# h2o/picotls

Hardware: AMD Instinct MI355X
Metric: AES-GCM seal+open GiB/s (device-resident), 16KiB & 1200B record batches (higher is better)
Workload: dtype u8

## Files before the change

### picotls_amd/csrc/engine/gcm_kernels.h

```cpp
#ifndef PTLS_MI355X_ENGINE_GCM_KERNELS_H
#define PTLS_MI355X_ENGINE_GCM_KERNELS_H

__device__ __forceinline__ u32 unit_mul(u32 steps, u32 log2, u32 cap)
{
    const u32 nc = (steps + (1u << log2) - 1) >> log2;
    return nc > cap ? (nc + cap - 1) / cap : 1u;
}
__device__ __forceinline__ u32 run_unit_cap(const BatchArgs &args)
{
    return args.w8_split ? (u32)W8_RUN_UNITS : (u32)CRUN_UNITS;
}

template <int FRAME = 0>
__device__ __forceinline__ bool record_ok(const BatchArgs &args, const ptls_mi355x_record_t &r)
{
    return r.len <= PTLS_MI355X_MAX_RECORD_LEN && gcm_aad_len<false, FRAME>(r) <= PTLS_MI355X_MAX_AAD_LEN &&
           r.key_idx < args.nkeys;
}

#ifndef SPREAD_MIN_BYTES
#define SPREAD_MIN_BYTES (512u << 10)
#endif
__device__ __forceinline__ bool spread_long(const BatchArgs &a, const ptls_mi355x_record_t &r)
{
// ... 517 lines not shown
            const u32 incl = carry + wave_incl_sum(np);
            if (t < 256) {
                plan[t] = incl - np;
                plan[256 + t] = e;
            }
            carry = (u32)__builtin_amdgcn_readlane((int)incl, 63);
        }
        if (lane == 0)
            plan[SPREAD_PLAN_CTL] = carry;
    }
    __syncthreads();
    const u32 P = __builtin_amdgcn_readfirstlane(plan[SPREAD_PLAN_CTL]);
    if (w >= P)
        return;
    auto piece_record = [&](u32 p) -> u32 {
        u32 lo = 0, hi = n;
        while (hi - lo > 1) {
            const u32 mid = (lo + hi) >> 1;
            if (plan[mid] <= p)
                lo = mid;
            else
                hi = mid;
        }
        return __builtin_amdgcn_readfirstlane(lo);
    };
    const u32 src8 = SPREAD_UNIT_STEPS == CHUNK_STEPS ? 8u : key_pow2_idx(3 + SPREAD_UNIT_LOG2);
    u32 loaded_key = args.multi_key ? args.recs[piece_record(w)].key_idx : 0u;
    if (wave >= EARLY_GHASH_WAVE)
        build_ghash_tables(lds, args.keys + loaded_key, 9, src8, 0, EARLY_GHASH_WAVE * 64, ENGINE_WG - EARLY_GHASH_WAVE * 64,
                           GHASH_WMASK);
    else
        build_aes_tables(lds, 0, EARLY_GHASH_WAVE * 64);
    __syncthreads();
    const u32 tsel_horner = 0x10000u + (u32)(G - 1) * GHASH_TABLE_BYTES, tsel_chunk = 0x10000u + 8u * GHASH_TABLE_BYTES;
    for (u32 p = w; p < P; p += nspare) {
        const u32 t = piece_record(p), s = p - plan[t], e = plan[256 + t], pbase = plan[t];
        const u32 np_t = (t + 1 < n ? plan[t + 1] : P) - pbase;
        const ptls_mi355x_record_t r = args.recs[t];
        const u32 kidx = args.multi_key ? __builtin_amdgcn_readfirstlane(r.key_idx) : 0u;
        if (kidx != loaded_key) {
            build_ghash_tables(lds, args.keys + kidx, 9, src8, 0, 0, 0, GHASH_WMASK);
            __syncthreads();
            loaded_key = kidx;
        }
        const KeyEntry *key = args.keys + kidx;
        u32 rk[NR + 1][4];
#pragma unroll
        for (int rr = 0; rr <= NR; ++rr)
#pragma unroll
            for (int c = 0; c < 4; ++c)
                rk[rr][c] = __builtin_amdgcn_readfirstlane(key->rk[rr][c]);
        const u32 iv0 = __builtin_amdgcn_readfirstlane(key->iv[0]), iv1 = __builtin_amdgcn_readfirstlane(key->iv[1]),
                  iv2 = __builtin_amdgcn_readfirstlane(key->iv[2]);
        const u32 steps = gcm_steps<OPEN, 0>(r), U = (steps + SPREAD_UNIT_STEPS - 1) / SPREAD_UNIT_STEPS;
        const u32 k0 = s << e, nu = min(U - k0, 1u << e);
        for (u32 uu0 = wave * 8; uu0 < nu; uu0 += ENGINE_WG / G) {
            const u32 lane = lane_here(), j = lane % G, uu = uu0 + lane / G, laneoff = (lane & 31) * 4;
            const bool valid = uu < nu;
            const u32 k = k0 + uu;
            u32 m_hi = 0, m_lo = 0;
            if (valid) {
                m_hi = steps - k * SPREAD_UNIT_STEPS;
                m_lo = k + 1 == U ? 0u : m_hi - SPREAD_UNIT_STEPS;
            }
            u32x4 acc;
            u32 okw;
            gcm_segment<NR, OPEN, 0, CT>(args, lds, rk, iv0, iv1, iv2, r, valid, m_lo, m_hi, j, laneoff, tsel_horner, acc, false,
                                         okw, false, CLDS_PART + 16u * uu);
            if (valid && j == G - 1)
                s_part[uu] = acc;
        }
        __syncthreads();
        const u32 mL = SPREAD_UNIT_LOG2 + e;
        const bool split = e >= 4 && mL <= 10 && (16u << e) <= GHASH_TABLE_BYTES;
        lds_u32x4 *s_sum = (lds_u32x4 *)(lds + CLDS_RUN1);
        const u32 tsel_ml = CLDS_PART + GHASH_TABLE_BYTES;
        if (split) {
            if (wave == 1)
                build_elem_table(lds, tsel_ml, u32x4{key->h[key_pow2_idx(mL)][0], key->h[key_pow2_idx(mL)][1],
                                                     key->h[key_pow2_idx(mL)][2], key->h[key_pow2_idx(mL)][3]}, 64, true);
            if (wave == 0) {
                const u32 lane = lane_here(), c = lane / G, L = 1u << (e - 3), ulo = c * L, uhi = min(ulo + L, nu);
                u32x4 g = {0, 0, 0, 0};
                if (ulo < uhi) {
                    g = s_part[uhi - 1];
                    for (u32 i = uhi - 1; i-- > ulo;)
                        g = gmul_combine(lds, g, tsel_chunk, lane) ^ s_part[i];
                }
                if (lane % G == 0)
                    s_sum[c] = g;
            }
            __syncthreads();
        }
        if (wave == 0) {
            const u32 lane = lane_here();
            u32x4 g;
            if (split) {
                g = s_sum[7];
                for (u32 c = 7; c-- > 0;)
                    g = gmul_combine(lds, g, tsel_ml, lane) ^ s_sum[c];
            } else {
                g = s_part[nu - 1];
                for (u32 i = nu - 1; i-- > 0;)
                    g = gmul_combine(lds, g, tsel_chunk, lane) ^ s_part[i];
            }
            if (lane == 0) {
                args.spread_part[pbase + s] = g;
                __threadfence();
                *s_flag = atomicAdd(args.spread_cnt + t, 1u) == np_t - 1;
            }
        }
        __syncthreads();
        if (*s_flag) {
            __threadfence();
            lds_u32x4 *s_m = (lds_u32x4 *)(lds + CLDS_PART + GHASH_TABLE_BYTES);
            const u32 m = 3 + SPREAD_UNIT_LOG2 + e, hi = m <= 10 ? key_pow2_idx(m) : 15u;
            if (threadIdx.x == 0)
                *s_m = u32x4{key->h[hi][0], key->h[hi][1], key->h[hi][2], key->h[hi][3]};
            __syncthreads();
            for (u32 i = 10; i < m; ++i) {
                build_elem_table(lds, CLDS_PART, *s_m);
                __syncthreads();
                const u32x4 sq = gmul_tab(lds, *s_m, CLDS_PART);
                __syncthreads();
                if (threadIdx.x == 0)
                    *s_m = sq;
                __syncthreads();
            }
            build_elem_table(lds, CLDS_PART, *s_m);
            __syncthreads();
            if (wave == 0) {
                const u32 lane = lane_here();
                const volatile u32x4 *vp = args.spread_part + pbase;
                u32x4 g = vp[np_t - 1];
                for (u32 i = np_t - 1; i-- > 0;)
                    g = gmul_tab(lds, g, CLDS_PART) ^ u32x4(vp[i]);
                if (lane == 0) {
                    if (OPEN) {
                        const u32x4 rt = *(const u32x4_u *)(args.in + r.in_off + r.len);
                        const u32x4 d = rt ^ g;
                        args.ok[t] = (d[0] | d[1] | d[2] | d[3]) == 0;
                    } else {
                        *(u32x4_u *)(args.out + r.out_off + r.len) = g;
                    }
                    args.spread_cnt[t] = 0;
                }
            }
        }
        __syncthreads();
    }
}


__device__ __noinline__ void w8_build_tables(lds_u8 *lds, const lds_u8 *keyp, u32 usrc, bool tree, u32 hpow)
{
    typedef __attribute__((address_space(3))) const KeyEntry lds_key_t;
    lds_key_t *key = (lds_key_t *)keyp;
    auto el = [&](u32 i) { return u32x4{key->h[i][0], key->h[i][1], key->h[i][2], key->h[i][3]}; };
    build_elem_table(lds, CLDS_PART, el(hpow), 0, false);
    build_elem_table(lds, W8_TAB_H, el(0), 64, !tree);
    if (tree)
        build_elem_table(lds, W8_TAB_COMB, el(1), 128, false);
    else if (usrc != 0xffffffffu)
        build_elem_table(lds, W8_TAB_COMB, el(usrc), 128, true);
    __syncthreads();
    build_h8_byte_table(lds, CLDS_PART);
    __syncthreads();
}

__device__ unsigned long long *g_kclock_buf;
__device__ unsigned int g_kclock_cap;
__device__ unsigned int g_kclock_n;

template <int NR, bool OPEN, int FRAME, bool CT = false, int EXT = 0>
__global__ __launch_bounds__(ENGINE_WG) __attribute__((amdgpu_waves_per_eu(ENGINE_WAVES_PER_SIMD, ENGINE_WAVES_PER_SIMD))) void gcm_chunked_kernel(BatchArgs args)
{
    extern __shared__ __attribute__((aligned(16))) uint8_t smem[];
    lds_u8 *lds = (lds_u8 *)smem;
    check_lds_base(smem);
    PROF_STAMP(tk);
    lds_u32x4 *s_part = (lds_u32x4 *)(lds + CLDS_PART);
    constexpr int G = ENGINE_G;
    constexpr int RPW = 64 / G;

    const u32 wave = threadIdx.x >> 6;
    const u32 tsel_horner = 0x10000u + (u32)(G - 1) * GHASH_TABLE_BYTES;
    constexpr bool W8K = EXT == 3 || EXT == 4 || EXT == 5;
    constexpr bool W8TREE = EXT == 3;
    const u32 tsel_chunk = W8K ? (u32)W8_TAB_COMB : 0x10000u + 8u * GHASH_TABLE_BYTES;

    const u64 n = args.nrecs, C = args.bounds != nullptr ? 0 : args.chunk;
    const u32 *slist = nullptr;
    u32 scnt = 0;
    if constexpr (W8TREE) {
        if (args.w8_split == 2 && args.w8_flags != nullptr) {
            scnt = args.w8_flags[(u64)blockIdx.x * W8_FLAG_WORDS];
            if (scnt == 0)
                return;
            if (scnt <= W8_SKIP_LIST)
                slist = args.w8_flags + (u64)blockIdx.x * W8_FLAG_WORDS + 1;
        }
    }
    unsigned long long *const kclock = ENGINE_HOOKS && blockIdx.x == 0 ? g_kclock_buf : nullptr;
    const u64 kc_t0 = kclock != nullptr ? __builtin_amdgcn_s_memtime() : 0ull;
    const u64 kc_r0 = kclock != nullptr ? __builtin_amdgcn_s_memrealtime() : 0ull;
    u32 skipped_w8 = 0;
    u32 runs_here = 0, g4_here = 0, mk_here = 0;
    constexpr bool SPREAD = FRAME == 0 && EXT == 1;
    if constexpr (SPREAD) {
        if (blockIdx.x >= n) {
            spread_pieces<NR, OPEN, CT>(args, blockIdx.x - (u32)n, gridDim.x - (u32)n);
            return;
        }
    }
    u64 beg = SPREAD ? (u64)blockIdx.x : args.bounds != nullptr ? args.bounds[blockIdx.x] : C != 0 ? min(n, (u64)blockIdx.x * C) : n * blockIdx.x / gridDim.x;
    u64 end = SPREAD ? (u64)blockIdx.x + 1 : args.bounds != nullptr ? args.bounds[blockIdx.x + 1] : C != 0 ? min(n, beg + C) : n * (blockIdx.x + 1) / gridDim.x;
    u64 cstart = beg;
    u32 sidx = 0;
    if constexpr (W8TREE) {
        if (slist != nullptr)
            beg = slist[0], end = slist[1];
    }
    u32 loaded_key = 0xffffffffu, loaded_usrc = 0xffffffffu;
    u32 loaded_w8 = 0;
    const ptls_mi355x_record_t *recs = args.recs;
    const u32 *perm = nullptr;
    if (args.perm_on != nullptr && *args.perm_on)
        recs = args.grouped, perm = args.perm;
    if (args.one_inline) {
        recs = (const ptls_mi355x_record_t *)(smem + CLDS_ONE);
        if (threadIdx.x < sizeof(ptls_mi355x_record_t) / 4)
            ((lds_u32 *)(lds + CLDS_ONE))[threadIdx.x] = ((const u32 *)&args.one)[threadIdx.x];
        __builtin_amdgcn_fence(__ATOMIC_SEQ_CST, "workgroup");
        __builtin_amdgcn_wave_barrier();
    }
    auto ok_at = [&](u64 i) -> u64 { return perm != nullptr ? (u64)perm[i] : i; };
    constexpr bool HPK = !OPEN && FRAME == 0 && EXT == 2;
    const bool with_hp = HPK && args.hp != nullptr;
    u64 hp_pos = 0;
    u32 hp_n = 0;
#define HP_PASS(p_, e_, tid_, nthr_)                                                                                    \
    do {                                                                                                                \
        if constexpr (HPK) {                                                                                            \
            if (args.hp_nr == 10)                                                                                       \
                hp_masks_pass<10>(args.hp, args.hp_keys, args.hp_nkeys, args.out, args.masks, (p_), (e_), perm, (tid_),  \
                                  (nthr_));                                                                             \
            else                                                                                                        \
                hp_masks_pass<14>(args.hp, args.hp_keys, args.hp_nkeys, args.out, args.masks, (p_), (e_), perm, (tid_),  \
                                  (nthr_));                                                                             \
        }                                                                                                               \
    } while (0)

    const bool early = !args.multi_key && !W8K;
    const u32 fixed_usrc = args.unit_log2 == CHUNK_LOG2 ? 8u : args.unit_log2 == 0 ? 7u : 8u + args.unit_log2;
    const bool early_combine = early && args.unit_log2 < CHUNK_LOG2;
    if (early && wave >= EARLY_GHASH_WAVE) {
        build_ghash_tables(lds, args.keys, early_combine ? 9u : 8u, fixed_usrc, 0, EARLY_GHASH_WAVE * 64,
                           ENGINE_WG - EARLY_GHASH_WAVE * 64, GHASH_WMASK);
    } else if (wave == 0) {
        if (beg < end)
            scan_run<OPEN, FRAME, true, EXT>(args, recs, beg, end, (lds_u32 *)(lds + CLDS_RUN0));
#if ENGINE_PROFILE
        if (threadIdx.x == 0)
            PROF_ADD(9, stamp() - tk), PROF_ADD(10, 1);
#endif
    } else {
        build_aes_tables(lds, 64, early ? EARLY_GHASH_WAVE * 64 : 0, W8K ? W8_AES_BASE : 0u);
#if ENGINE_PROFILE
        if (threadIdx.x == 64)
            PROF_ADD(8, stamp() - tk);
#endif
    }
    __syncthreads();

    if (early)
        loaded_key = 0, loaded_usrc = early_combine ? fixed_usrc : 0xffffffffu;

    u32 rb = 0;
    for (u64 pos = beg; pos < end;) {
        PROF_STAMP(t0);
        lds_u32 *rs = (lds_u32 *)(lds + (rb ? CLDS_RUN1 : CLDS_RUN0));
        lds_u32 *rs_next = (lds_u32 *)(lds + (rb ? CLDS_RUN0 : CLDS_RUN1));
        lds_u32 *s_ubase = rs + RUN_UBASE_OFF, *s_done = rs + RUN_DONE_OFF, *s_front = rs + RUN_FRONT_OFF;
        const u32 key_idx = __builtin_amdgcn_readfirstlane(rs[RC_KEY]);
        const u32 run_n = __builtin_amdgcn_readfirstlane(rs[RC_N]);
        const bool whole_run = __builtin_amdgcn_readfirstlane(rs[RC_WHOLE]);
        const u32 total_units = __builtin_amdgcn_readfirstlane(rs[RC_UNITS]);
        const u32 nhuge = __builtin_amdgcn_readfirstlane(rs[RC_HUGE]);
        const u32 mk_n = EXT == 5 ? __builtin_amdgcn_readfirstlane(rs[RC_MK]) : 0u;
        const u32 ulog2 = __builtin_amdgcn_readfirstlane(rs[RC_LOG2]), ustep = 1u << ulog2;
        const u32 usrc = ustep == CHUNK_STEPS ? 8u : ulog2 == 0 ? 7u : 8u + ulog2;
        const u32 nfull = total_units - run_n;
        const u64 run_end = pos + run_n;
        u64 nxt = run_end, nxt_end = end, nxt_cstart = cstart;
        if (C != 0 && run_end >= end) {
            nxt_cstart = cstart + (u64)gridDim.x * C;
            nxt = min(n, nxt_cstart);
            nxt_end = min(n, nxt_cstart + C);
        }
        if constexpr (W8TREE) {
            if (slist != nullptr) {
                if (sidx + 1 < scnt) {
                    nxt = slist[2 * sidx + 2];
                    nxt_end = slist[2 * sidx + 3];
                } else {
                    nxt = nxt_end = 0;
                }
                ++sidx;
            }
        }
        PROF_STAMP(t1);

        if (W8K && args.w8_split == 2) {
            const bool tree = whole_run &&
                              __builtin_amdgcn_readfirstlane(gcm_steps<OPEN, FRAME>(recs[pos]) >= W8_MIN_STEPS ? 1u : 0u) != 0;
            if (tree != W8TREE) {
                if constexpr (!W8TREE) {
                    const bool fits = end <= 0xffffffffull;
                    if (args.w8_flags != nullptr && threadIdx.x == 0 && skipped_w8 < W8_SKIP_LIST && fits) {
                        u32 *f = args.w8_flags + (u64)blockIdx.x * W8_FLAG_WORDS + 1 + 2 * skipped_w8;
                        f[0] = (u32)pos, f[1] = (u32)end;
                    }
                    skipped_w8 = fits ? skipped_w8 + 1 : W8_SKIP_LIST + 1;
                }
                if (wave == 0 && nxt < nxt_end)
                    scan_run<OPEN, FRAME, false, EXT>(args, recs, nxt, nxt_end, rs_next);
                __syncthreads();
                pos = nxt, end = nxt_end, cstart = nxt_cstart;
                rb ^= 1;
                continue;
            }
        }
        const bool whole = W8TREE || whole_run;
        if (key_idx >= args.nkeys) {
            if (OPEN)
                for (u64 t = pos + threadIdx.x; t < run_end; t += blockDim.x)
                    args.ok[ok_at(t)] = 0;
            if (wave == 0 && nxt < nxt_end)
                scan_run<OPEN, FRAME, false, EXT>(args, recs, nxt, nxt_end, rs_next);
            __syncthreads();
            if (with_hp) {
                if (hp_n != 0)
                    HP_PASS(hp_pos, hp_pos + hp_n, threadIdx.x, blockDim.x);
                HP_PASS(pos, run_end, threadIdx.x, blockDim.x);
                hp_n = 0;
            }
            pos = nxt, end = nxt_end, cstart = nxt_cstart;
            rb ^= 1;
            continue;
        }
        ++runs_here;
        typedef __attribute__((address_space(3))) const KeyEntry lds_key_t;
        lds_key_t *key = (lds_key_t *)(rs + RUN_KEY_OFF);
        constexpr bool w8run = W8K;
        const bool g4run = W8K && !W8TREE && whole;
        const u32 w8mode = !w8run ? 0u : W8TREE ? 2u : g4run ? 3u : 1u;
        const bool key_new = key_idx != loaded_key;
        if (mk_n != 0) {
            static_assert(ENGINE_WG >= 2 * MK_SLOTS * 128, "a table per 128 threads");
            const u32 t = threadIdx.x >> 7, slot = t >> 1;
            if (slot < mk_n) {
                lds_key_t *kp = mk_key(rs, slot);
                const u32 el = (t & 1) ? 0u : 3u;
                build_elem_table_w4(lds, slot * MK_SLOT_BYTES + (t & 1) * GHASH_TABLE_BYTES,
                                    u32x4{kp->h[el][0], kp->h[el][1], kp->h[el][2], kp->h[el][3]}, 128u * t);
            }
            __syncthreads();
            loaded_key = 0xffffffffu;
            loaded_usrc = 0xffffffffu;
            loaded_w8 = 4;
        } else if (w8run && (key_new || loaded_w8 != w8mode)) {
            w8_build_tables(lds, (const lds_u8 *)key, whole ? 0xffffffffu : usrc, w8mode == 2, w8mode == 3 ? 3u : 7u);
            loaded_key = key_idx;
            loaded_usrc = whole ? 0xffffffffu : usrc;
            loaded_w8 = w8mode;
            if (threadIdx.x == 0)
                PROF_ADD(7, 1);
        } else if (w8run && !whole && usrc != loaded_usrc) {
            build_elem_table(lds, W8_TAB_COMB, u32x4{key->h[usrc][0], key->h[usrc][1], key->h[usrc][2], key->h[usrc][3]}, 0, true);
            __syncthreads();
            loaded_usrc = usrc;
        } else if (!w8run && (key_idx != loaded_key || loaded_w8 || (!whole && usrc != loaded_usrc))) {
            build_ghash_tables(lds, key, 9, usrc, key_idx != loaded_key || loaded_w8 ? 0u : 8u, 0, 0, GHASH_WMASK);
            __syncthreads();
            loaded_key = key_idx;
            loaded_usrc = usrc;
            loaded_w8 = 0;
            if (threadIdx.x == 0)
                PROF_ADD(7, 1);
        }
#if ENGINE_PROFILE
        unsigned long long t2 = stamp();
#endif
        if (EXT == 5 && mk_n != 0) {
            ++mk_here;
            if (wave == ENGINE_WG / 64 - 1) {
                u32 claim = 0;
                if (lane_here() == 0)
                    claim = atomicAdd((u32 *)&rs[RC_CLAIM], 1u) == 0;
                PROF_STAMP(ts0);
                if (__builtin_amdgcn_readfirstlane(claim) && nxt < nxt_end)
                    scan_run<OPEN, FRAME, false, EXT>(args, recs, nxt, nxt_end, rs_next);
#if ENGINE_PROFILE
                if (lane_here() == 0)
                    PROF_ADD(15, stamp() - ts0);
#endif
            }
            {
                constexpr u32 G4 = 4;
                for (;;) {
                    u32 cb = 0;
                    if (lane_here() == 0)
                        cb = atomicAdd((u32 *)&rs[RC_NEXT], 1u);
                    cb = __builtin_amdgcn_readfirstlane(cb);
                    if (cb >= total_units)
                        break;
                    PROF_STAMP(tc0);
                    const u32 e = __builtin_amdgcn_readfirstlane(rs[RUN_UBASE_OFF + cb]);
                    const u32 mk_first = e & 0xffu, mk_cnt = (e >> 8) & 0xffu, slot = e >> 16;
                    lds_key_t *kp = mk_key(rs, slot);
                    u32 rkm[NR + 1][4];
#pragma unroll
                    for (int r = 0; r <= NR; ++r)
#pragma unroll
                        for (int c = 0; c < 4; ++c)
                            rkm[r][c] = __builtin_amdgcn_readfirstlane(kp->rk[r][c]);
                    const u32 mv0 = __builtin_amdgcn_readfirstlane(kp->iv[0]), mv1 = __builtin_amdgcn_readfirstlane(kp->iv[1]),
                              mv2 = __builtin_amdgcn_readfirstlane(kp->iv[2]);
                    u32x4 acc;
                    u32 okw;
                    {
                        const u32 lane = lane_here(), j = lane % G4, qd = lane / G4;
                        const u32 laneoff = (lane & 31) * 4 | W8_AES_BASE;
                        const bool valid = qd < mk_cnt;
                        ptls_mi355x_record_t r = {};
                        if (valid)
                            r = recs[pos + mk_first + qd];
                        const bool live = valid && record_ok<FRAME>(args, r);
                        if (!live)
                            r.len = 0, r.aad_len = 0, r.flags = 0;
                        const u32 ekslot = CLDS_PART + 16u * (threadIdx.x / G4);
                        gcm_segment<NR, OPEN, FRAME, CT, true, (int)G4, true>(
                            args, lds, rkm, mv0, mv1, mv2, r, live, 0u, live ? 2u * gcm_steps<OPEN, FRAME>(r) : 0u, j, laneoff, 0u, acc,
                            true, okw, true, ekslot, false, mk_kslot(slot));
                    }
                    asm volatile("" ::: "memory");
                    const u32 qd = lane_here() / G4;
                    if (OPEN && okw <= 1 && qd < mk_cnt)
                        args.ok[ok_at(pos + mk_first + qd)] = (uint8_t)okw;
#if ENGINE_PROFILE
                    if (lane_here() == 0)
                        PROF_ADD(13, stamp() - tc0), PROF_ADD(14, 1);
#endif
                }
            }
        } else {
#if ENGINE_PROFILE
        t2 = stamp();
#endif
        u32 rk[NR + 1][4];
#pragma unroll
        for (int r = 0; r <= NR; ++r)
#pragma unroll
            for (int c = 0; c < 4; ++c)
                rk[r][c] = __builtin_amdgcn_readfirstlane(key->rk[r][c]);
        const u32 iv0 = __builtin_amdgcn_readfirstlane(key->iv[0]), iv1 = __builtin_amdgcn_readfirstlane(key->iv[1]),
                  iv2 = __builtin_amdgcn_readfirstlane(key->iv[2]);

        auto unit_of = [&](u32 u, u32 &lo, u32 &first, u32 &unc, u32 &k_back) {
            lo = u, first = u, unc = 1, k_back = 0;
            if (whole)
                return;
            if (u < nhuge || u >= nhuge + nfull) {
                lo = s_front[u < nhuge ? u : u - nfull];
                first = s_ubase[lo];
                unc = s_ubase[lo + 1] - first;
                k_back = unc - 1;
            } else {
                const u32 f = u - nhuge;
                u32 hi = run_n;
                lo = 0;
                while (hi - lo > 1) {
                    const u32 mid = (lo + hi) >> 1;
                    if (s_ubase[mid] - mid <= f)
                        lo = mid;
                    else
                        hi = mid;
                }
                first = s_ubase[lo];
                unc = s_ubase[lo + 1] - first;
                k_back = f - (first - lo);
            }
        };
        bool g4done = false;
        if constexpr (W8K && !W8TREE) {
            if (g4run) {
                constexpr u32 G4 = 4, RPW4 = 64 / G4;
                ++g4_here;
                for (;;) {
                    u32 ub = 0;
                    if (lane_here() == 0)
                        ub = atomicAdd((u32 *)&rs[RC_NEXT], RPW4);
                    ub = __builtin_amdgcn_readfirstlane(ub);
                    if (ub >= total_units)
                        break;
                    u32x4 acc;
                    u32 okw;
                    {
                        const u32 lane = lane_here(), j = lane % G4, u = ub + lane / G4;
                        const u32 laneoff = (lane & 31) * 4 | W8_AES_BASE;
                        const bool valid = u < total_units;
                        u32 lo, first, unc, k_back;
                        unit_of(valid ? u : 0u, lo, first, unc, k_back);
                        ptls_mi355x_record_t r = {};
                        if (valid)
                            r = recs[pos + lo];
                        const bool live = valid && record_ok<FRAME>(args, r);
                        if (valid && !live) {
                            r.len = 0, r.aad_len = 0, r.flags = 0;
                            if (OPEN && j == 0)
                                args.ok[ok_at(pos + lo)] = 0;
                        }
                        const u32 steps = gcm_steps<OPEN, FRAME>(r);
                        u32 m_hi = steps, m_lo = 0;
                        if (!whole) {
                            const u32 ulen = unit_mul(steps, ulog2, run_unit_cap(args)) * ustep;
                            m_hi = steps - k_back * ulen;
                            m_lo = k_back + 1 == unc ? 0u : m_hi - ulen;
                        }
                        if (!live)
                            m_lo = m_hi = 0;
                        const u32 ekslot = CLDS_PART + 16u * (whole ? threadIdx.x / G4 : first + unc - 1);
                        gcm_segment<NR, OPEN, FRAME, CT, true, (int)G4>(args, lds, rk, iv0, iv1, iv2, r, live, 2u * m_lo, 2u * m_hi,
                                                                      j, laneoff, tsel_horner, acc, unc == 1, okw, whole,
                                                                      ekslot, false);
                    }
                    asm volatile("" ::: "memory");
                    const u32 lane = lane_here(), j = lane % G4, u = ub + lane / G4;
                    if (u >= total_units)
                        continue;
                    u32 lo, first, unc, k_back;
                    unit_of(u, lo, first, unc, k_back);
                    if (OPEN && okw <= 1)
                        args.ok[ok_at(pos + lo)] = (uint8_t)okw;
                }
                g4done = true;
            }
        }
        if (!g4done)
        for (;;) {
            u32 ub = 0;
            if (lane_here() == 0)
                ub = atomicAdd((u32 *)&rs[RC_NEXT], (u32)RPW);
            ub = __builtin_amdgcn_readfirstlane(ub);
            if (ub >= total_units) {
                if (with_hp && hp_n != 0) {
                    u32 m = 0;
                    if (lane_here() == 0)
                        m = atomicAdd((u32 *)&rs[RC_HPNEXT], (u32)HP_ITEM);
                    m = __builtin_amdgcn_readfirstlane(m);
                    if (m < hp_n) {
                        HP_PASS(hp_pos + m, hp_pos + min(hp_n, m + (u32)HP_ITEM), lane_here(), 64u);
                        continue;
                    }
                }
                break;
            }
            u32x4 acc;
            u32 okw;
            {
                const u32 lane = lane_here(), j = lane % G, slot = lane / G, laneoff = (lane & 31) * 4 | (W8K ? W8_AES_BASE : 0u);
                const u32 u = ub + slot;
                const bool valid = u < total_units;
                u32 lo, first, unc, k_back;
                unit_of(valid ? u : 0u, lo, first, unc, k_back);
                ptls_mi355x_record_t r = {};
                if (valid)
                    r = recs[pos + lo];
                const bool spread = SPREAD && valid && spread_long(args, r);
                const bool live = valid && !spread && record_ok<FRAME>(args, r);
                if (valid && !live) {
                    r.len = 0, r.aad_len = 0, r.flags = 0;
                    if (OPEN && j == 0 && !spread)
                        args.ok[ok_at(pos + lo)] = 0;
                }
                const u32 steps = gcm_steps<OPEN, FRAME>(r);
                const u32 mul = whole ? 1u : unit_mul(steps, ulog2, run_unit_cap(args));
                u32 m_hi = steps, m_lo = 0;
                if (!whole) {
                    const u32 ulen = mul * ustep;
                    m_hi = steps - k_back * ulen;
                    m_lo = k_back + 1 == unc ? 0u : m_hi - ulen;
                }
                if (!live)
                    m_lo = m_hi = 0;
                const u32 ekslot = CLDS_PART + 16u * (whole ? threadIdx.x / G : first + unc - 1);
                gcm_segment<NR, OPEN, FRAME, CT, W8K>(args, lds, rk, iv0, iv1, iv2, r, live, m_lo, m_hi, j, laneoff, tsel_horner,
                                                      acc, unc == 1, okw, whole, ekslot, W8TREE);
            }
            asm volatile("" ::: "memory");
            const u32 lane = lane_here(), j = lane % G, u = ub + lane / G;
            if (u >= total_units)
                continue;
            u32 lo, first, unc, k_back;
            unit_of(u, lo, first, unc, k_back);
            if (OPEN && okw <= 1)
                args.ok[ok_at(pos + lo)] = (uint8_t)okw;
#if ENGINE_PROFILE
            PROF_STAMP(tc0);
#endif
            if (unc > 1) {
                u32 last = 0;
                if (j == G - 1) {
                    s_part[first + unc - 1 - k_back] = acc;
                    __threadfence_block();
                    last = atomicAdd((u32 *)&s_done[lo], 1u) == unc - 1;
                }
                last = dpp_bcast7(last, lane);
                if (last) {
                    const ptls_mi355x_record_t r = recs[pos + lo];
                    const u32 mul = unit_mul(gcm_steps<OPEN, FRAME>(r), ulog2, run_unit_cap(args));
                    const GroupWs k = group_ws(tsel_chunk, lane);
                    const u32 q = j >> 1;
                    const u32x4 z = {0, 0, 0, 0};
                    u32 gs = ((const lds_u32 *)(s_part + first))[q];
                    for (u32 i = 1; i < unc; ++i) {
                        for (u32 t = 0; t < mul; ++t)
                            gs = gmul_group_ws(lds, gs, k, z, lane);
                        gs ^= ((const lds_u32 *)(s_part + first + i))[q];
                    }
                    const u32x4 g = group_gather(gs, lane);
                    const u32x4 tag = g;
                    if (j != G - 1) {
                    } else if (OPEN) {
                        const u32x4 rt = *(const u32x4_u *)(args.in + r.in_off + frame_in_skip<OPEN, FRAME>() +
                                                            gcm_text_len<OPEN, FRAME>(r));
                        const u32x4 d = rt ^ tag;
                        args.ok[ok_at(pos + lo)] = (d[0] | d[1] | d[2] | d[3]) == 0;
                    } else {
                        *(u32x4_u *)(args.out + r.out_off + frame_out_skip<OPEN, FRAME>() + gcm_text_len<OPEN, FRAME>(r)) = tag;
                    }
                }
            }
#if ENGINE_PROFILE
            if (lane_here() == 0)
                PROF_ADD(11, stamp() - tc0), PROF_ADD(12, 1);
#endif
        }
        }
        u32 claim = 0;
        if (lane_here() == 0)
            claim = atomicAdd((u32 *)&rs[RC_CLAIM], 1u) == 0;
#if ENGINE_PROFILE
        PROF_STAMP(tsc);
#endif
        if (__builtin_amdgcn_readfirstlane(claim) && nxt < nxt_end)
            scan_run<OPEN, FRAME, false, EXT>(args, recs, nxt, nxt_end, rs_next);
        PROF_STAMP(tw);
        __syncthreads();
        if (with_hp)
            hp_pos = pos, hp_n = run_n;
        PROF_STAMP(t3);
#if ENGINE_PROFILE
        if (lane_here() == 0)
            PROF_ADD(4, t3 - tw);
        if (lane_here() == 0 && mk_n == 0 && __builtin_amdgcn_readfirstlane(claim) && nxt < nxt_end)
            PROF_ADD(13, tw - tsc), PROF_ADD(14, t3 - tw);
        if (threadIdx.x == 0) {
            PROF_ADD(0, t1 - t0);
            PROF_ADD(1, t2 - t1);
            PROF_ADD(2, t3 - t2);
            PROF_ADD(5, total_units);
            PROF_ADD(6, 1);
            if (pos == beg)
                PROF_ADD(3, t0 - tk);
        }
#endif
        pos = nxt, end = nxt_end, cstart = nxt_cstart;
        rb ^= 1;
    }
    if (with_hp && hp_n != 0)
        HP_PASS(hp_pos, hp_pos + hp_n, threadIdx.x, blockDim.x);
    if constexpr (W8K && !W8TREE) {
        if (args.w8_split == 2 && args.w8_flags != nullptr && threadIdx.x == 0)
            args.w8_flags[(u64)blockIdx.x * W8_FLAG_WORDS] = min(skipped_w8, (u32)W8_SKIP_LIST + 1);
    }
    if (ENGINE_HOOKS && threadIdx.x == 0) {
        if (runs_here != 0)
            atomicAdd(&g_ext_runs[blockIdx.x % EXT_RUN_ROWS][EXT == 5 ? 4 : EXT], (unsigned long long)runs_here);
        if (g4_here != 0)
            atomicAdd(&g_ext_runs[blockIdx.x % EXT_RUN_ROWS][7], (unsigned long long)g4_here);
        if (EXT == 5 && mk_here != 0)
            atomicAdd(&g_ext_runs[blockIdx.x % EXT_RUN_ROWS][6], (unsigned long long)mk_here);
    }
    if (kclock != nullptr && threadIdx.x == 0) {
        const u64 t1 = __builtin_amdgcn_s_memtime(), r1 = __builtin_amdgcn_s_memrealtime();
        const u32 i = atomicAdd(&g_kclock_n, 1u);
        if (i < g_kclock_cap) {
            kclock[4 * i + 0] = kc_t0, kclock[4 * i + 1] = t1;
            kclock[4 * i + 2] = kc_r0, kclock[4 * i + 3] = r1;
        }
    }
    publish_done(args.done_flag, args.done_token);
#undef HP_PASS
}

#endif
```

### picotls_amd/csrc/engine/ghash.h

```cpp
#ifndef PTLS_MI355X_ENGINE_GHASH_H
#define PTLS_MI355X_ENGINE_GHASH_H


__device__ __forceinline__ u32x4 gmul_tab(const lds_u8 *, u32x4 a, u32 tsel)
{
    u32x4 acc = {0, 0, 0, 0};
#pragma unroll
    for (int q = 0; q < 4; ++q) {
        const u32 w = a[q];
        const u32 hi = w & 0xf0f0f0f0u, lo = (w << 4) & 0xf0f0f0f0u;
#pragma unroll
        for (int k = 0; k < 4; ++k) {
            const u32 sel = 0x0c020100u | (4u + k);
            const u32x4 e0 = lds_load128(__builtin_amdgcn_perm(hi, tsel, sel) + (8 * q + 2 * k) * 256);
            const u32x4 e1 = lds_load128(__builtin_amdgcn_perm(lo, tsel, sel) + (8 * q + 2 * k + 1) * 256);
#pragma unroll
            for (int c = 0; c < 4; ++c)
                acc[c] = xor3(acc[c], e0[c], e1[c]);
        }
    }
    return acc;
}


// ... 222 lines not shown
__device__ __forceinline__ GroupWs group_ws(u32 tsel, u32 lane)
{
    GroupWs k;
    const u32 W = wtab_lane_base(tsel, lane), h16 = 16u * (lane & 1), f4 = 4u * ((lane >> 2) & 3);
#pragma unroll
    for (u32 i = 0; i < 4; ++i) {
        k.Wi[i] = W ^ (i << 4);
        k.sh[i] = h16 + (f4 ^ (4u * (i ^ 1u)));
        asm volatile("" : "+v"(k.Wi[i]), "+v"(k.sh[i]));
    }
    return k;
}

__device__ __forceinline__ u32 group_scatter(u32x4 t, u32 lane)
{
    const bool b = (lane & 4) != 0, c = (lane & 2) != 0;
    const u32 k0 = b ? t[2] : t[0], k1 = b ? t[3] : t[1], s0 = b ? t[0] : t[2], s1 = b ? t[1] : t[3];
    const u32 m0 = k0 ^ (u32)__builtin_amdgcn_update_dpp(0, (int)s0, 0x141, 0xF, 0xF, false);
    const u32 m1 = k1 ^ (u32)__builtin_amdgcn_update_dpp(0, (int)s1, 0x141, 0xF, 0xF, false);
    const u32 kk = c ? m1 : m0, ss = c ? m0 : m1;
    const u32 m = kk ^ (u32)__builtin_amdgcn_update_dpp(0, (int)ss, 0x4E, 0xF, 0xF, false);
    return m ^ (u32)__builtin_amdgcn_update_dpp(0, (int)m, 0xB1, 0xF, 0xF, false);
}

__device__ __forceinline__ u32x4 group_gather(u32 g, u32 lane)
{
    const u32 a = (u32)__builtin_amdgcn_update_dpp(0, (int)g, 0x00, 0xF, 0xF, false);
    const u32 b = (u32)__builtin_amdgcn_update_dpp(0, (int)g, 0xAA, 0xF, 0xF, false);
    const u32 am = (u32)__builtin_amdgcn_update_dpp(0, (int)a, 0x141, 0xF, 0xF, false);
    const u32 bm = (u32)__builtin_amdgcn_update_dpp(0, (int)b, 0x141, 0xF, 0xF, false);
    const bool hi = (lane & 4) != 0;
    return u32x4{hi ? am : a, hi ? bm : b, hi ? a : am, hi ? b : bm};
}

__device__ __forceinline__ u32 group_dword(u32x4 v, u32 lane)
{
    const u32 q = (lane & 7) >> 1;
    return q == 0 ? v[0] : q == 1 ? v[1] : q == 2 ? v[2] : v[3];
}

__device__ __forceinline__ u32x4 group_ws_terms(u32 ga, const GroupWs &k, u32x4 x)
{
    u32x4 e[4];
#pragma unroll
    for (u32 i = 0; i < 4; ++i)
        e[i] = lds_load128((CT_PROBE_CONST ? 0u : __builtin_amdgcn_ubfe(ga, k.sh[i], 4u) << 8) + k.Wi[i]);
    u32x4 t;
#pragma unroll
    for (int c = 0; c < 4; ++c)
        t[c] = xor3(xor3(e[0][c], e[1][c], e[2][c]), e[3][c], x[c]);
    return t;
}

__device__ __forceinline__ u32 gmul_group_ws(const lds_u8 *, u32 ga, const GroupWs &k, u32x4 x, u32 lane)
{
    return group_scatter(group_ws_terms(ga, k, x), lane);
}

__device__ __forceinline__ u32x4 gmul_group_ws_full(const lds_u8 *, u32 ga, const GroupWs &k)
{
    u32x4 t = group_ws_terms(ga, k, u32x4{0, 0, 0, 0});
#pragma unroll
    for (int c = 0; c < 4; ++c)
        t[c] = dpp_xor8(t[c]);
    return t;
}

#ifndef W8_END_SCATTER
#define W8_END_SCATTER 1
#endif

__device__ __forceinline__ u32x4 w8_lane_end(const lds_u8 *lds, u32x4 v, u32 lane, u32 rank)
{
    static_assert(ENGINE_G == 8, "a chain over 8 lanes");
    const u32x4 z = {0, 0, 0, 0};
#if W8_END_SCATTER
    const GroupWs k = group_ws(W8_TAB_H, lane);
    u32 g = group_scatter(rank == 0 ? v : z, lane);
#pragma unroll
    for (u32 r = 1; r < 8; ++r)
        g = gmul_group_ws(lds, g, k, rank == r ? v : z, lane);
    return gmul_group_ws_full(lds, g, k);
#else
    u32x4 g;
#pragma unroll
    for (int c = 0; c < 4; ++c)
        g[c] = dpp_xor8(rank == 0 ? v[c] : 0u);
#pragma unroll
    for (u32 r = 1; r < 8; ++r)
        g = gmul_group_w_add(lds, g, W8_TAB_H, lane, rank == r ? v : z);
    return gmul_group_w(lds, g, W8_TAB_H, lane);
#endif
}

struct Group4Ws {
    u32 Wi[8];
    u32 sh[8];
};
__device__ __forceinline__ Group4Ws group4_ws(u32 tsel, u32 lane)
{
    Group4Ws k;
    const u32 y = lane & 3, f = (lane >> 1) & 7;
    const u32 B = tsel + (y >> 1) * 4096u + (y & 1) * 128u + f * 16u;
#pragma unroll
    for (u32 i = 0; i < 8; ++i) {
        k.Wi[i] = B ^ (i << 4);
        k.sh[i] = 4u * ((i ^ f) ^ 1u);
        asm volatile("" : "+v"(k.Wi[i]), "+v"(k.sh[i]));
    }
    return k;
}
__device__ __forceinline__ u32x4 group4_ws_terms(u32 ga, const Group4Ws &k, u32x4 x)
{
    u32x4 t = x;
#pragma unroll
    for (u32 i = 0; i < 8; i += 2) {
        const u32x4 e0 = lds_load128((__builtin_amdgcn_ubfe(ga, k.sh[i], 4u) << 8) + k.Wi[i]);
        const u32x4 e1 = lds_load128((__builtin_amdgcn_ubfe(ga, k.sh[i + 1], 4u) << 8) + k.Wi[i + 1]);
#pragma unroll
        for (int c = 0; c < 4; ++c)
            t[c] = xor3(t[c], e0[c], e1[c]);
    }
    return t;
}
__device__ __forceinline__ u32 group4_scatter(u32x4 t, u32 lane)
{
    const bool b = (lane & 2) != 0, c = (lane & 1) != 0;
    const u32 k0 = b ? t[2] : t[0], k1 = b ? t[3] : t[1], s0 = b ? t[0] : t[2], s1 = b ? t[1] : t[3];
    const u32 m0 = k0 ^ (u32)__builtin_amdgcn_update_dpp(0, (int)s0, 0x4E, 0xF, 0xF, false);
    const u32 m1 = k1 ^ (u32)__builtin_amdgcn_update_dpp(0, (int)s1, 0x4E, 0xF, 0xF, false);
    const u32 kk = c ? m1 : m0, ss = c ? m0 : m1;
    return kk ^ (u32)__builtin_amdgcn_update_dpp(0, (int)ss, 0xB1, 0xF, 0xF, false);
}
__device__ __forceinline__ u32x4 group4_allreduce(u32x4 t)
{
#pragma unroll
    for (int c = 0; c < 4; ++c) {
        t[c] ^= (u32)__builtin_amdgcn_update_dpp(0, (int)t[c], 0x4E, 0xF, 0xF, false);
        t[c] ^= (u32)__builtin_amdgcn_update_dpp(0, (int)t[c], 0xB1, 0xF, 0xF, false);
    }
    return t;
}
__device__ __forceinline__ u32x4 w8_lane_end4(const lds_u8 *, u32x4 v, u32 lane, u32 rank, u32 htab = W8_TAB_H)
{
    const u32x4 z = {0, 0, 0, 0};
    const Group4Ws k = group4_ws(htab, lane);
    u32 g = group4_scatter(rank == 0 ? v : z, lane);
#pragma unroll
    for (u32 r = 1; r < 4; ++r)
        g = group4_scatter(group4_ws_terms(g, k, rank == r ? v : z), lane);
    return group4_allreduce(group4_ws_terms(g, k, z));
}

__device__ __forceinline__ u32x4 w8_tree_end(const lds_u8 *lds, u32x4 v, u32 lane, u32 rank)
{
    const u32 rot = ((lane & 7u) - rank) & 7u;
#pragma unroll 1
    for (u32 lv = 0; lv < 3; ++lv) {
        const u32 k = 1u << lv;
        u32x4 y = gmul_tab(lds, v, lv == 0 ? (u32)W8_TAB_H : (u32)W8_TAB_COMB);
        if (lv == 2)
            y = gmul_tab(lds, y, W8_TAB_COMB);
        const bool hi = (rank & k) != 0;
        const u32x4 send = hi ? v : y;
        const int src = (int)(((lane & ~7u) | (((rank ^ k) + rot) & 7u)) * 4u);
        u32x4 recv;
#pragma unroll
        for (int c = 0; c < 4; ++c)
            recv[c] = (u32)__builtin_amdgcn_ds_bpermute(src, (int)send[c]);
        v = hi ? (recv ^ v) : (y ^ recv);
    }
    return gmul_tab(lds, v, W8_TAB_H);
}

#endif
```

### picotls_amd/csrc/engine/segment.h

```cpp
#ifndef PTLS_MI355X_ENGINE_SEGMENT_H
#define PTLS_MI355X_ENGINE_SEGMENT_H

template <int NR, bool OPEN, int FRAME = 0, bool CT = false, bool W8 = false, int GG = ENGINE_G, bool MK4 = false>
__device__ __forceinline__ void gcm_segment(const BatchArgs &args, const lds_u8 *lds, const u32 (&rk)[NR + 1][4], u32 iv0,
                                            u32 iv1, u32 iv2, const ptls_mi355x_record_t &r, bool valid, u32 m_lo,
                                            u32 m_hi, u32 j, u32 laneoff, u32 tsel_horner, u32x4 &acc, bool finish,
                                            u32 &okw, bool aligned, u32 ekslot = 0, bool w8tree = false,
                                            u32 mk_kslot = MK_NONE)
{
    constexpr int G = GG;
    static_assert(G == 8 || (G == 4 && W8), "8-lane groups, or 4-lane groups in the W8 kernels");
#if ENGINE_PROFILE
    const unsigned long long tsg0 = stamp();
#endif
    constexpr int GS = G == 8 ? 3 : 2;
    W8Lane w8 = {};
    if constexpr (W8)
        w8 = w8_lane(lane_here());
    static_assert(!MK4 || (W8 && G == 4), "MK runs are 4-lane W8 runs");
    MK4Lane mk4 = {};
    if constexpr (MK4)
        mk4 = mk4_lane(lane_here());
    auto horner = [&](u32x4 t) -> u32x4 {
        if constexpr (MK4)
// ... 134 lines not shown
            }
        } else if (is_len) {
            u32 Ah = A, Lh = L;
            asm volatile("" : "+v"(Ah), "+v"(Lh));
            const u64 abits = (u64)Ah * 8, cbits = (u64)Lh * 8;
            X[0] = bswap32((u32)(abits >> 32));
            X[1] = bswap32((u32)abits);
            X[2] = bswap32((u32)(cbits >> 32));
            X[3] = bswap32((u32)cbits);
            *(lds_u32x4 *)(const_cast<lds_u8 *>(lds) + ekslot) = ks;
        }
        return X;
    };

    const int D0 = P + (int)na;
    const int nbf = (int)(Lsrc >> 4);
    const int ms = (D0 + G - 1) / G;
    const int me = nbf + D0 >= G ? (nbf + D0 - G) / G : -1;
    int sa = max(ms, (int)m_lo) - (int)m_lo;
    int sb = min(me - 1, m_first_last - 1) + 1 - (int)m_lo;
    if (!valid || m_hi <= m_lo)
        sa = 1, sb = 0;
    sa = wave_smax_perg<G>(sa);
    sb = wave_smin_perg<G>(sb);

    auto progress_prio = [&](u32 left) {
        if constexpr (TREE_PRIO_BAND && W8) {
            if (w8tree) {
                const u32 q = left / TREE_PRIO_BAND;
                const u32 lvl = q >= 3 ? 3u : q;
                if (lvl == 3)
                    __builtin_amdgcn_s_setprio(3);
                else if (lvl == 2)
                    __builtin_amdgcn_s_setprio(2);
                else if (lvl == 1)
                    __builtin_amdgcn_s_setprio(1);
                else
                    __builtin_amdgcn_s_setprio(0);
                return;
            }
        }
        if constexpr (PROGRESS_PRIO && W8) {
            if (w8tree)
                return;
            if (left > 3u * PROGRESS_PRIO)
                __builtin_amdgcn_s_setprio(3);
            else if (left > 2u * PROGRESS_PRIO)
                __builtin_amdgcn_s_setprio(2);
            else if (left > 1u * PROGRESS_PRIO)
                __builtin_amdgcn_s_setprio(1);
            else
                __builtin_amdgcn_s_setprio(0);
        }
    };
#if ENGINE_PROFILE
    const unsigned long long tsg1 = stamp();
    unsigned long long tsteady = 0;
#endif
    for (u32 s0 = 0; s0 < Smax; ++s0) {
        progress_prio(Smax - s0);
        if ((int)s0 == sa && sb > sa) {
#if ENGINE_PROFILE
            const unsigned long long tst0 = stamp();
#endif
            const int b0 = (int)(j + G * (m_lo + (u32)sa)) - D0;
            u32 off = 16u * (u32)b0;
            u32 ctr = (u32)b0 + 2;
            constexpr bool LINE = OPEN && G == 4;
            constexpr bool PAIR = G == 4 && !LINE;
            u32x4 held = {0, 0, 0, 0};
            bool have = false;
            u32x4 held2 = {0, 0, 0, 0};
            bool late = false;
            uint8_t *dst_l = dst;
            if constexpr (LINE) {
                late = j > (((u32)(uintptr_t)(dst + off) >> 4) & 3u);
                dst_l = dst - (late ? 64 : 0);
            }
            const bool holder = G == 8 && ((u32)(uintptr_t)(dst + off) & 127u) < 16u * j;
            const bool pair8 = G == 8 && W8 && FRAME == 0 && !aligned && __any(holder);
            for (int s = sa; s < sb; ++s) {
                if ((s & 3) == 0)
                    progress_prio(Smax - (u32)s);
                cur = nxt;
                nxt = *(const u32x4_u *)(src + off + 16 * G);
                u32 st[1][4] = {{n0, n1, n2, bswap32(ctr) ^ rk[0][3]}};
                if ((ctr >> 8) != cc1_key) {
                    cc1 = ctr_cache1_init<NR>(lds, laneoff, rk, n0, n1, n2, st[0][3]);
                    cc1_key = ctr >> 8;
                }
                aes_ctr_cached1<NR>(lds, laneoff, rk, cc1, st);
                __builtin_amdgcn_sched_barrier(0);
                const u32x4 o = cur ^ u32x4{st[0][0], st[0][1], st[0][2], st[0][3]};
                if constexpr (LINE) {
                    const bool first = (((u32)(uintptr_t)(dst + off)) & 64u) == 0;
                    if (!first)
                        held2 = o;
                    if (first == late) {
                        uint8_t *p = dst_l + off;
                        if (s >= sa + 1 + (int)late)
                            *(u32x4_u *)(p - 64) = held;
                        if (!late || s > sa)
                            *(u32x4_u *)p = held2;
                    }
                    if (first)
                        held = o;
                } else if constexpr (PAIR) {
                    if ((((uintptr_t)(dst + off)) & 64u) == 0 && s + 1 < sb) {
                        held = o;
                        have = true;
                    } else {
                        if (have)
                            *(u32x4_u *)(dst + off - 16 * G) = held;
                        *(u32x4_u *)(dst + off) = o;
                        have = false;
                    }
                } else if (pair8) {
                    if (have)
                        *(u32x4_u *)(dst + off - 16 * G) = held;
                    have = holder && s + 1 < sb;
                    if (have)
                        held = o;
                    else
                        *(u32x4_u *)(dst + off) = o;
                } else {
                    *(u32x4_u *)(dst + off) = o;
                }
                __builtin_amdgcn_sched_barrier(0);
                if constexpr (W8)
                    acc = horner(acc ^ (OPEN ? cur : o));
                else
                    acc = gmul_tab(lds, acc ^ (OPEN ? cur : o), tsel_horner);
                __builtin_amdgcn_sched_barrier(0);
                ctr += G;
                off += 16 * G;
            }
            if constexpr (LINE) {
                uint8_t *p = dst + off - 16 * G;
                if ((((u32)(uintptr_t)p) & 64u) == 0) {
                    *(u32x4_u *)p = held;
                } else if (late) {
                    *(u32x4_u *)p = held2;
                    if (sb - 1 > sa)
                        *(u32x4_u *)(p - 64) = held;
                }
            }
            s0 = (u32)sb;
#if ENGINE_PROFILE
            tsteady += stamp() - tst0;
#endif
        }
        const u32 m0 = m_lo + s0;
        const int lg = (int)(j + G * m0) - P;
        const bool wave_ks = G != 4 || __any(m0 < m_hi && lg >= (int)na && lg <= (int)(na + nb)) != 0;
        u32 st[1][4];
        setup_step(m0, st, wave_ks);
        if (wave_ks)
            aes_ctr_cached1<NR>(lds, laneoff, rk, cc1, st);
        __builtin_amdgcn_sched_barrier(0);
        const u32x4 X = finish_step(m0, u32x4{st[0][0], st[0][1], st[0][2], st[0][3]});
        __builtin_amdgcn_sched_barrier(0);
        const bool last_here = (int)m0 == m_last;
        const u32x4 t = acc ^ X;
        u32x4 prod = t;
        if (s0 + 1 < Smax) {
            if constexpr (W8)
                prod = horner(t);
            else
                prod = gmul_tab(lds, t, tsel_horner);
            if (last_here)
                prod = t;
        }
        if ((int)m0 <= m_last)
            acc = prod;
        __builtin_amdgcn_sched_barrier(0);
    }
    if constexpr ((PROGRESS_PRIO != 0 || TREE_PRIO_BAND != 0) && W8)
        __builtin_amdgcn_s_setprio(0);
#if ENGINE_PROFILE
    const unsigned long long tsg2 = stamp();
#endif

    static_assert(G == 8 || W8, "dpp_xor8 reduces groups of 8 lanes");
    u32x4 rt = {0, 0, 0, 0};
    if (OPEN && finish && valid && j == jl)
        rt = *(const u32x4_u *)(src + L);
    if constexpr (W8) {
        const u32 rank = valid ? (u32)G - e_last : j;
        if constexpr (G == 4)
            acc = w8_lane_end4(lds, acc, lane_here(), rank, MK4 ? mk_htab(mk_kslot) : (u32)W8_TAB_H);
        else if (w8tree)
            acc = w8_tree_end(lds, acc, lane_here(), rank);
        else
            acc = w8_lane_end(lds, acc, lane_here(), rank);
        if (valid && m_hi * G >= N && j == jl)
            acc ^= u32x4(*(const lds_u32x4 *)(lds + ekslot));
    } else {
        const u32 rank = valid ? (u32)G - e_last : j;
        acc = coop_last_powers(lds, acc, lane_here(), (j - rank) & (G - 1));
#pragma unroll
        for (int c = 0; c < 4; ++c)
            acc[c] = dpp_xor8(acc[c]);
        acc = gmul_group_w(lds, acc, LDS_AES_BYTES, lane_here());
        if (valid && m_hi * G >= N && j == jl)
            acc ^= u32x4(*(const lds_u32x4 *)(lds + ekslot));
    }
    okw = 2;
    if (finish && valid && j == jl) {
        const u32x4 tag = acc;
        if (OPEN) {
            const u32x4 d = rt ^ tag;
            okw = (d[0] | d[1] | d[2] | d[3]) == 0;
        } else {
            *(u32x4_u *)(dst + L) = tag;
        }
    }
#if ENGINE_PROFILE
    if (W8 && !w8tree && lane_here() == 0) {
        const unsigned long long tsg3 = stamp();
        PROF_ADD(16, tsg1 - tsg0), PROF_ADD(17, tsg2 - tsg1), PROF_ADD(18, tsg3 - tsg2), PROF_ADD(19, 1);
        PROF_ADD(20, Smax), PROF_ADD(21, sb > sa ? (u32)(sb - sa) : 0u), PROF_ADD(22, tsteady);
    }
#endif
}

#endif
```

Baseline: 1267.

## Drop W8 tree reduction, interleave unit claims, skip idle keystream waves

Removes the tree-based end reduction (w8_tree_end) and its extra H^2 combine table, so W8TREE runs use the standard lane-end reduction and share table builds with regular W8 runs. Under W8TREE, each wave's claimed units are strided across blocks of RPW*RPW instead of being contiguous, which changes how records are spread over waves. For non-TLS12 tree runs, the keystream step is also gated by a wave-wide __any check so waves with no live lanes skip AES work. Together these aim to cut table-build cost and wasted keystream work, at the risk of worse locality and a longer serial reduction.

```diff
diff --git a/picotls_amd/csrc/engine/gcm_kernels.h b/picotls_amd/csrc/engine/gcm_kernels.h
--- a/picotls_amd/csrc/engine/gcm_kernels.h
+++ b/picotls_amd/csrc/engine/gcm_kernels.h
@@ -693,16 +693,14 @@
 }
 
 
-__device__ __noinline__ void w8_build_tables(lds_u8 *lds, const lds_u8 *keyp, u32 usrc, bool tree, u32 hpow)
+__device__ __noinline__ void w8_build_tables(lds_u8 *lds, const lds_u8 *keyp, u32 usrc, u32 hpow)
 {
     typedef __attribute__((address_space(3))) const KeyEntry lds_key_t;
     lds_key_t *key = (lds_key_t *)keyp;
     auto el = [&](u32 i) { return u32x4{key->h[i][0], key->h[i][1], key->h[i][2], key->h[i][3]}; };
     build_elem_table(lds, CLDS_PART, el(hpow), 0, false);
-    build_elem_table(lds, W8_TAB_H, el(0), 64, !tree);
-    if (tree)
-        build_elem_table(lds, W8_TAB_COMB, el(1), 128, false);
-    else if (usrc != 0xffffffffu)
+    build_elem_table(lds, W8_TAB_H, el(0), 64, true);
+    if (usrc != 0xffffffffu)
         build_elem_table(lds, W8_TAB_COMB, el(usrc), 128, true);
     __syncthreads();
     build_h8_byte_table(lds, CLDS_PART);
@@ -895,7 +893,7 @@
         lds_key_t *key = (lds_key_t *)(rs + RUN_KEY_OFF);
         constexpr bool w8run = W8K;
         const bool g4run = W8K && !W8TREE && whole;
-        const u32 w8mode = !w8run ? 0u : W8TREE ? 2u : g4run ? 3u : 1u;
+        const u32 w8mode = !w8run ? 0u : g4run ? 3u : 1u;
         const bool key_new = key_idx != loaded_key;
         if (mk_n != 0) {
             static_assert(ENGINE_WG >= 2 * MK_SLOTS * 128, "a table per 128 threads");
@@ -911,7 +909,7 @@
             loaded_usrc = 0xffffffffu;
             loaded_w8 = 4;
         } else if (w8run && (key_new || loaded_w8 != w8mode)) {
-            w8_build_tables(lds, (const lds_u8 *)key, whole ? 0xffffffffu : usrc, w8mode == 2, w8mode == 3 ? 3u : 7u);
+            w8_build_tables(lds, (const lds_u8 *)key, whole ? 0xffffffffu : usrc, w8mode == 3 ? 3u : 7u);
             loaded_key = key_idx;
             loaded_usrc = whole ? 0xffffffffu : usrc;
             loaded_w8 = w8mode;
@@ -1033,6 +1031,13 @@
                 k_back = f - (first - lo);
             }
         };
+        auto claim_unit = [&](u32 ub, u32 slot) -> u32 {
+            if constexpr (W8TREE)
+                return (ub & ~63u) + ((ub >> 3) & 7u) + (u32)RPW * slot;
+            else
+                return ub + slot;
+        };
+        static_assert(RPW == 8, "claim_unit deals blocks of RPW * RPW units");
         bool g4done = false;
         if constexpr (W8K && !W8TREE) {
             if (g4run) {
@@ -1094,7 +1099,7 @@
             if (lane_here() == 0)
                 ub = atomicAdd((u32 *)&rs[RC_NEXT], (u32)RPW);
             ub = __builtin_amdgcn_readfirstlane(ub);
-            if (ub >= total_units) {
+            if (claim_unit(ub, 0) >= total_units) {
                 if (with_hp && hp_n != 0) {
                     u32 m = 0;
                     if (lane_here() == 0)
@@ -1111,7 +1116,7 @@
             u32 okw;
             {
                 const u32 lane = lane_here(), j = lane % G, slot = lane / G, laneoff = (lane & 31) * 4 | (W8K ? W8_AES_BASE : 0u);
-                const u32 u = ub + slot;
+                const u32 u = claim_unit(ub, slot);
                 const bool valid = u < total_units;
                 u32 lo, first, unc, k_back;
                 unit_of(valid ? u : 0u, lo, first, unc, k_back);
@@ -1140,7 +1145,7 @@
                                                       acc, unc == 1, okw, whole, ekslot, W8TREE);
             }
             asm volatile("" ::: "memory");
-            const u32 lane = lane_here(), j = lane % G, u = ub + lane / G;
+            const u32 lane = lane_here(), j = lane % G, u = claim_unit(ub, lane / G);
             if (u >= total_units)
                 continue;
             u32 lo, first, unc, k_back;
diff --git a/picotls_amd/csrc/engine/ghash.h b/picotls_amd/csrc/engine/ghash.h
--- a/picotls_amd/csrc/engine/ghash.h
+++ b/picotls_amd/csrc/engine/ghash.h
@@ -398,25 +398,4 @@
     return group4_allreduce(group4_ws_terms(g, k, z));
 }
 
-__device__ __forceinline__ u32x4 w8_tree_end(const lds_u8 *lds, u32x4 v, u32 lane, u32 rank)
-{
-    const u32 rot = ((lane & 7u) - rank) & 7u;
-#pragma unroll 1
-    for (u32 lv = 0; lv < 3; ++lv) {
-        const u32 k = 1u << lv;
-        u32x4 y = gmul_tab(lds, v, lv == 0 ? (u32)W8_TAB_H : (u32)W8_TAB_COMB);
-        if (lv == 2)
-            y = gmul_tab(lds, y, W8_TAB_COMB);
-        const bool hi = (rank & k) != 0;
-        const u32x4 send = hi ? v : y;
-        const int src = (int)(((lane & ~7u) | (((rank ^ k) + rot) & 7u)) * 4u);
-        u32x4 recv;
-#pragma unroll
-        for (int c = 0; c < 4; ++c)
-            recv[c] = (u32)__builtin_amdgcn_ds_bpermute(src, (int)send[c]);
-        v = hi ? (recv ^ v) : (y ^ recv);
-    }
-    return gmul_tab(lds, v, W8_TAB_H);
-}
-
 #endif
diff --git a/picotls_amd/csrc/engine/segment.h b/picotls_amd/csrc/engine/segment.h
--- a/picotls_amd/csrc/engine/segment.h
+++ b/picotls_amd/csrc/engine/segment.h
@@ -310,7 +310,7 @@
         }
         const u32 m0 = m_lo + s0;
         const int lg = (int)(j + G * m0) - P;
-        const bool wave_ks = G != 4 || __any(m0 < m_hi && lg >= (int)na && lg <= (int)(na + nb)) != 0;
+        const bool wave_ks = (G != 4 && !(w8tree && !TLS12)) || __any(m0 < m_hi && lg >= (int)na && lg <= (int)(na + nb)) != 0;
         u32 st[1][4];
         setup_step(m0, st, wave_ks);
         if (wave_ks)
@@ -347,8 +347,6 @@
         const u32 rank = valid ? (u32)G - e_last : j;
         if constexpr (G == 4)
             acc = w8_lane_end4(lds, acc, lane_here(), rank, MK4 ? mk_htab(mk_kslot) : (u32)W8_TAB_H);
-        else if (w8tree)
-            acc = w8_tree_end(lds, acc, lane_here(), rank);
         else
             acc = w8_lane_end(lds, acc, lane_here(), rank);
         if (valid && m_hi * G >= N && j == jl)
```

New measurement: 1290, median of 6. 1.8% higher.
